# IamJerryXu/Multimodal-Diagnosis-HAM-Spine

Hardware: AMD Instinct MI355X
Metric: training images/sec, ResNet50+BERT-base 224px bs32 (higher is better)
Workload: dtype bf16; 1 GPU; C2: ResNet50 + BERT-base(L=128) + cross-attention FusionModule + MLP head, 224x224, batch 32 per GPU, CE(label_smoothing=0.02), fused AdamW, train-mode BatchNorm and dropout; per_gpu_batch=32, global_batch=32, seq_len=128, params=134897991, parallelism=dp1

## Files before the change

### include/hamspine.h

```cpp
#ifndef HAMSPINE_H
#define HAMSPINE_H

#include <stdint.h>

#ifdef __cplusplus
extern "C" {
#endif

typedef int hs_status;
enum { HS_OK = 0, HS_ERR_ARG = 1, HS_ERR_HIP = 2, HS_ERR_UNSUPPORTED = 3 };
enum { HS_F32 = 0, HS_BF16 = 1 };

const char* hs_last_error(void);
int hs_version(void);
int hs_device_ok(void);


enum {
    HS_A_KC = 0,
    HS_A_RC = 1,
    HS_A_CONV = 2,
    HS_A_DGRAD = 3
};
enum {
// ... 194 lines not shown
                             float* const* exp_avg_sq, const int64_t* n, float lr, float beta1, float beta2, float eps,
                             float weight_decay, int32_t step, int32_t decoupled, float grad_scale, void* stream);
hs_status hs_adam_step_multi_shadow(int32_t count, float* const* params, const float* const* grads, float* const* exp_avg,
                                    float* const* exp_avg_sq, void* const* bf16_shadow, const int64_t* n, float lr, float beta1,
                                    float beta2, float eps, float weight_decay, int32_t step, int32_t decoupled,
                                    float grad_scale, void* stream);
hs_status hs_wgrad_group_begin(void* stream);
hs_status hs_wgrad_group_end(void* stream);
hs_status hs_wgrad_defer_begin(void* stream);
hs_status hs_wgrad_defer_suspend(void* stream);
int32_t hs_wgrad_defer_open(void* stream);
int32_t hs_wgrad_defer_pending(void* stream);
int64_t hs_wgrad_defer_ws_bytes(void* stream);
hs_status hs_wgrad_defer_flush(void* stream, void* ws, int64_t ws_bytes);
hs_status hs_wgrad_defer_abort(void* stream);
void hs_wgrad_defer_counters(int64_t* out);
hs_status hs_weight_shadow_set(const float* w, void* bf16);
void hs_weight_shadow_clear(void);

hs_status hs_sgd_step_multi(int32_t count, float* const* params, const float* const* grads, float* const* momentum_buf,
                            const int64_t* n, float lr, float momentum, float weight_decay, int32_t nesterov, int32_t first,
                            float grad_scale, void* stream);

#define HS_GRADCLIP_MAX 128
hs_status hs_grad_sumsq_multi(int32_t count, const float* const* grads, const int64_t* n, double* partials, void* stream);
int64_t hs_grad_norm_partials(int32_t count, const int64_t* n);
hs_status hs_grad_norm_finish(const double* partials, int64_t n_partials, float max_norm, int32_t skip_nonfinite, float* rec,
                              void* stream);
hs_status hs_grad_scale_multi(int32_t count, float* const* grads, const int64_t* n, const float* rec, void* stream);
hs_status hs_adam_step_multi_clip(int32_t count, float* const* params, const float* const* grads, float* const* exp_avg,
                                  float* const* exp_avg_sq, void* const* bf16_shadow, const int64_t* n, float lr, float beta1,
                                  float beta2, float eps, float weight_decay, int32_t step, int32_t decoupled, float grad_scale,
                                  const float* rec, void* stream);
hs_status hs_sgd_step_multi_clip(int32_t count, float* const* params, const float* const* grads, float* const* momentum_buf,
                                 const int64_t* n, float lr, float momentum, float weight_decay, int32_t nesterov, int32_t first,
                                 float grad_scale, const float* rec, void* stream);

#define HS_MUON_MAX 32
#define HS_MUON_PARTIALS 256
hs_status hs_muon_prepare_multi(int32_t dtype, int32_t count, float* const* momentum, const float* const* grads,
                                void* const* packed, const int32_t* rows, const int32_t* cols, float beta, float* partials,
                                void* stream);
hs_status hs_muon_orthogonalize(int32_t dtype, int32_t count, int32_t rows, int32_t cols, void* X, void* ws, int64_t ws_bytes,
                                void* stream);
int64_t hs_muon_ws_bytes(int32_t dtype, int32_t count, int32_t rows, int32_t cols);
hs_status hs_muon_apply_multi(int32_t dtype, int32_t count, float* const* params, void* const* bf16_shadow,
                              const void* const* packed, const int32_t* rows, const int32_t* cols, const float* scale,
                              float lr, float weight_decay, void* stream);

hs_status hs_select_token_fwd(int32_t dtype, const void* x, float* out, int32_t B, int32_t Nt, int32_t H, int32_t t,
                              void* stream);
hs_status hs_select_token_bwd(int32_t dtype, const float* dy, void* dx, int32_t B, int32_t Nt, int32_t H, int32_t t,
                              void* stream);
hs_status hs_concat2(const float* a, int32_t Ha, const float* b, int32_t Hb, float* out, int64_t rows, void* stream);
hs_status hs_split2(const float* g, float* da, int32_t Ha, float* db, int32_t Hb, int64_t rows, void* stream);
hs_status hs_concat2_t(int32_t dtype, const void* a, int32_t Ha, const void* b, int32_t Hb, void* out, int64_t rows,
                       void* stream);
hs_status hs_split2_t(int32_t dtype, const void* g, void* da, int32_t Ha, void* db, int32_t Hb, int64_t rows, void* stream);
hs_status hs_mul(const float* a, const float* b, float* out, int64_t rows, int32_t cols, int32_t b_mode, void* stream);
hs_status hs_rowdot(const float* a, const float* b, float* out, int32_t rows, int32_t cols, void* stream);
hs_status hs_kl_rows(const float* p, const float* q, float* out, const float* w, float* dp, float* dq, int32_t rows,
                     int32_t cols, float eps, void* stream);
hs_status hs_dot(const float* a, const float* b, float* out, int64_t n, void* stream);
hs_status hs_sigmoid_fwd(const float* x, float* out, int64_t n, void* stream);
hs_status hs_sigmoid_bwd(const float* dy, const float* y, float* dx, int64_t n, void* stream);
hs_status hs_softmax_entropy(const float* logits, const float* g, float* ent, float* dlogits, int32_t rows, int32_t C,
// ... 377 lines not shown
```

### multimodal-diagnosis-ham-spine_amd/hamspine/_lib.py

```python
import collections
import ctypes as C
import os
import re

_HERE = os.path.dirname(os.path.abspath(__file__))
LIB_PATH = os.path.join(_HERE, "libhamspine_hip.so")
HEADER_PATH = os.path.normpath(os.path.join(_HERE, "..", "..", "include", "hamspine.h"))

HS_OK = 0


class HamspineError(RuntimeError):
    pass


_SCALARS = {"int": C.c_int32, "int32_t": C.c_int32, "hs_status": C.c_int32, "int64_t": C.c_int64, "uint64_t": C.c_uint64,
            "float": C.c_float}
_POINTEES = {"void", "char", "double", "uint8_t", "int16_t", "uint16_t", *_SCALARS}

Header = collections.namedtuple("Header", "constants structs prototypes")


def _symbols(text):
    return sorted(set(re.findall(r"\b(hs_[a-z0-9_]+)\s*\(", re.sub(r"/\*.*?\*/", "", text, flags=re.S))))
# ... 120 lines not shown
}
_ALL_STRUCT_NAMES = {**_STRUCT_NAMES, **_LATER_STRUCT_NAMES}
if set(_header.structs) != set(_ALL_STRUCT_NAMES):
    raise HamspineError(f"{HEADER_PATH}: structs without a Python name, or the reverse: {set(_header.structs) ^ set(_ALL_STRUCT_NAMES)}")
_classes = {}
for _c, _fields in _header.structs.items():
    _classes[_c] = type(_ALL_STRUCT_NAMES[_c], (C.Structure,), {"_fields_": [
        (f, _ctype(t, _classes, False) * n if n else _ctype(t, _classes, False)) for f, t, n in _fields]})
globals().update({_ALL_STRUCT_NAMES[_c]: _cls for _c, _cls in _classes.items()})


def abi_structs():
    return list(enumerate(_classes[c] for c in _STRUCT_NAMES))


def later_abi_structs():
    return list(enumerate((_classes[c] for c in _LATER_STRUCT_NAMES), start=len(_STRUCT_NAMES)))


def _const(*names):
    return [_header.constants["HS_" + n] for n in names]


if _const("OK") != [HS_OK]:
    raise HamspineError("HS_OK of the header is not 0")
HS_ERR_ARG, HS_ERR_HIP, HS_ERR_UNSUPPORTED = _const("ERR_ARG", "ERR_HIP", "ERR_UNSUPPORTED")
HS_F32, HS_BF16 = _const("F32", "BF16")
A_KC, A_RC, A_CONV, A_DGRAD = _const("A_KC", "A_RC", "A_CONV", "A_DGRAD")
B_KC, B_RC, B_WDGRAD, B_CONV = _const("B_KC", "B_RC", "B_WDGRAD", "B_CONV")
ACT_NONE, ACT_RELU, ACT_GELU = _const("ACT_NONE", "ACT_RELU", "ACT_GELU")
MUL_NONE, MUL_GELU_GRAD, MUL_RELU_MASK = _const("MUL_NONE", "MUL_GELU_GRAD", "MUL_RELU_MASK")
CAST_MAX, ADAM_MAX, MUON_MAX, MUON_PARTIALS = _const("CAST_MAX", "ADAM_MAX", "MUON_MAX", "MUON_PARTIALS")
GRADCLIP_MAX, = _const("GRADCLIP_MAX")
RESNET_MAX_BLOCKS, RESNET_MAX_TAPS, BERT_MAX_LAYERS = _const("RESNET_MAX_BLOCKS", "RESNET_MAX_TAPS", "BERT_MAX_LAYERS")
JPEG_GEOM, JPEG_CHUNK, JPEG_MAX_COMPONENTS = _const("JPEG_GEOM", "JPEG_CHUNK", "JPEG_MAX_COMPONENTS")
JPEG_STATUS = {v: k[len("HS_JPEG_ERR_"):] for k, v in _header.constants.items() if k.startswith("HS_JPEG_ERR_")}

_lib = None


def lib():
    global _lib
    if _lib is None:
        if not os.path.exists(LIB_PATH):
            raise HamspineError(
                f"{LIB_PATH} not found: build it with `python __graft_entry__.py build` "
                "(hipcc --offload-arch=gfx950). There is no CPU fallback.")
        l = C.CDLL(LIB_PATH)
        missing = [n for n in _header.prototypes if not hasattr(l, n)]
        if missing:
            raise HamspineError(f"{LIB_PATH} lacks declared symbols: {missing}")
        for n, (ret, params) in _header.prototypes.items():
            getattr(l, n).restype = None if ret == "void" else _ctype(ret, _classes, True)
            getattr(l, n).argtypes = [_ctype(t, _classes, True) for t in params]
        _lib = l
    return _lib


def check(status, what=""):
    if status != HS_OK:
        msg = lib().hs_last_error().decode("utf-8", "replace")
        raise HamspineError(f"{what} failed (status {status}): {msg}")
```

### multimodal-diagnosis-ham-spine_amd/hamspine/csrc/elem.hip

```cpp
#include <algorithm>
#include "hs_internal.h"

namespace hs {

static inline int grid_for(long long n, int cap = 4096) {
    long long b = (n + 255) / 256;
    if (b > cap) b = cap;
    if (b < 1) b = 1;
    return (int)b;
}

template <typename T>
__global__ __launch_bounds__(256) void maxpool_fwd_kernel(const T* __restrict__ x, T* __restrict__ y,
                                                          unsigned char* __restrict__ idx, int N, int H, int W, int C,
                                                          int P, int Q, int ks, int st, int pad) {
    constexpr int E = Chunk<T>::N;
    const int cg = C / E;
    const long long total = (long long)N * P * Q * cg;
    for (long long i = (long long)blockIdx.x * 256 + threadIdx.x; i < total; i += (long long)gridDim.x * 256) {
        const int c = (int)(i % cg);
        long long t = i / cg;
        const int q = (int)(t % Q);
        t /= Q;
        const int p = (int)(t % P);
        const int n = (int)(t / P);
        float best[E];
        unsigned char bi[E];
#pragma unroll
        for (int e = 0; e < E; ++e) {
            best[e] = -INFINITY;
            bi[e] = 0;
        }
        for (int r = 0; r < ks; ++r) {
            const int h = p * st - pad + r;
// ... 946 lines not shown
    if (threadIdx.x == 0) loss_out[0] = tn / td;
    if (!dlogits) return;
    for (int r = wv; r < B; r += nwv) {
        const float* z = logits + (long long)r * C;
        float mx = -INFINITY;
        for (int c = lane; c < C; c += 64) mx = fmaxf(mx, z[c]);
        mx = wave_max(mx);
        float se = 0.f;
        for (int c = lane; c < C; c += 64) se += __expf(z[c] - mx);
        const float inv = 1.f / wave_sum(se);
        const int y = (int)labels[r];
        const float wy = weight ? weight[y] : 1.f;
        float wsum = 0.f;
        for (int c = lane; c < C; c += 64) wsum += weight ? weight[c] : 1.f;
        wsum = wave_sum(wsum);
        for (int c = lane; c < C; c += 64) {
            const float p = __expf(z[c] - mx) * inv;
            const float wc = weight ? weight[c] : 1.f;
            float g = (1.f - smoothing) * wy * (p - (c == y ? 1.f : 0.f)) + smoothing / (float)C * (wsum * p - wc);
            dlogits[(long long)r * C + c] = g / td;
        }
    }
}

struct AdamTable {
    float* p[HS_ADAM_MAX];
    const float* g[HS_ADAM_MAX];
    float* m[HS_ADAM_MAX];
    float* v[HS_ADAM_MAX];
    long long n[HS_ADAM_MAX];
    bf16_t* h[HS_ADAM_MAX];
};
__device__ __forceinline__ const float* clip_rec(const float* rec) { return rec; }
template <bool CLIP, typename... Rec>
__global__ __launch_bounds__(256) void adam_multi_kernel(const AdamTable t, float lr, float beta1, float beta2, float eps,
                                                         float wd, float bc1, float bc2_sqrt, int decoupled,
                                                         float grad_scale, Rec... rec) {
    static_assert(sizeof...(Rec) == (CLIP ? 1 : 0), "the record comes with CLIP and only with it");
    float clip = 1.f;
    if constexpr (CLIP) {
        const float* r = clip_rec(rec...);
        if (r[3] != 0.f) return;
        clip = r[1];
    }
    const int e = blockIdx.y;
    float* p = t.p[e];
    const float* g = t.g[e];
    float* m = t.m[e];
    float* v = t.v[e];
    const long long n = t.n[e];
    auto upd = [&](float& pi, float gi, float& mi, float& vi) {
        gi *= grad_scale;
        if constexpr (CLIP) gi *= clip;
        if (decoupled) pi *= 1.f - lr * wd;
        else gi += wd * pi;
        mi = beta1 * mi + (1.f - beta1) * gi;
        vi = beta2 * vi + (1.f - beta2) * gi * gi;
        const float denom = sqrtf(vi) / bc2_sqrt + eps;
        pi = pi - (lr / bc1) * (mi / denom);
    };
    bf16_t* h = t.h[e];
    const bool al = (((uintptr_t)p | (uintptr_t)g | (uintptr_t)m | (uintptr_t)v) & 15) == 0 && (((uintptr_t)h) & 7) == 0;
    const long long n4 = al ? n / 4 : 0;
    for (long long i = (long long)blockIdx.x * 256 + threadIdx.x; i < n4; i += (long long)gridDim.x * 256) {
        f32x4 pv = ((f32x4*)p)[i], mv = ((f32x4*)m)[i], vv = ((f32x4*)v)[i];
        const f32x4 gv = ((const f32x4*)g)[i];
#pragma unroll
        for (int k = 0; k < 4; ++k) {
            float pi = pv[k], mi = mv[k], vi = vv[k];
            upd(pi, gv[k], mi, vi);
            pv[k] = pi; mv[k] = mi; vv[k] = vi;
        }
        ((f32x4*)p)[i] = pv;
        ((f32x4*)m)[i] = mv;
        ((f32x4*)v)[i] = vv;
        if (h) ((bf16x4*)h)[i] = bf16x4{(bf16_t)pv[0], (bf16_t)pv[1], (bf16_t)pv[2], (bf16_t)pv[3]};
    }
    for (long long i = n4 * 4 + (long long)blockIdx.x * 256 + threadIdx.x; i < n; i += (long long)gridDim.x * 256) {
        float pi = p[i], mi = m[i], vi = v[i];
        upd(pi, g[i], mi, vi);
        p[i] = pi; m[i] = mi; v[i] = vi;
        if (h) h[i] = (bf16_t)pi;
    }
}

template <bool CLIP, typename... Rec>
__global__ __launch_bounds__(256) void sgd_multi_kernel(const AdamTable t, float lr, float momentum, float wd, int nesterov,
                                                        int first, float grad_scale, Rec... rec) {
    static_assert(sizeof...(Rec) == (CLIP ? 1 : 0), "the record comes with CLIP and only with it");
    float clip = 1.f;
    if constexpr (CLIP) {
        const float* r = clip_rec(rec...);
        if (r[3] != 0.f) return;
        clip = r[1];
    }
    const int e = blockIdx.y;
    float* p = t.p[e];
    const float* g = t.g[e];
    float* buf = t.m[e];
    const long long n = t.n[e];
    for (long long i = (long long)blockIdx.x * 256 + threadIdx.x; i < n; i += (long long)gridDim.x * 256) {
        float gi = g[i] * grad_scale;
        if constexpr (CLIP) gi *= clip;
        const float pi = p[i];
        if (wd != 0.f) gi += wd * pi;
        if (buf) {
            const float b = first ? gi : momentum * buf[i] + gi;
            buf[i] = b;
            gi = nesterov ? gi + momentum * b : b;
        }
        p[i] = pi - lr * gi;
    }
}

#define DISPATCH_T(dtype, fn, ...) ((dtype) == HS_BF16 ? fn<bf16_t>(__VA_ARGS__) : fn<float>(__VA_ARGS__))
// ... 590 lines not shown
            t.m[i] = exp_avg[base + i];
            t.v[i] = exp_avg_sq[base + i];
            t.n[i] = n[base + i];
            t.h[i] = bf16_shadow ? (bf16_t*)bf16_shadow[base + i] : nullptr;
            mx = std::max<long long>(mx, t.n[i]);
        }
        const int gx = (int)std::min<long long>(std::max<long long>((mx + 4095) / 4096, 1), 256);
        if (rec)
            hipLaunchKernelGGL((adam_multi_kernel<true, const float*>), dim3(gx, cnt), dim3(256), 0, (hipStream_t)stream, t, lr, beta1, beta2, eps,
                               weight_decay, bc1, bc2s, decoupled, grad_scale, rec);
        else
            hipLaunchKernelGGL(adam_multi_kernel<false>, dim3(gx, cnt), dim3(256), 0, (hipStream_t)stream, t, lr, beta1, beta2, eps,
                               weight_decay, bc1, bc2s, decoupled, grad_scale);
        HS_LAUNCH_CHECK();
    }
    return HS_OK;
}
hs_status hs_adam_step_multi_shadow(int32_t count, float* const* params, const float* const* grads, float* const* exp_avg,
                                    float* const* exp_avg_sq, void* const* bf16_shadow, const int64_t* n, float lr, float beta1,
                                    float beta2, float eps, float weight_decay, int32_t step, int32_t decoupled,
                                    float grad_scale, void* stream) {
    return adam_step(count, params, grads, exp_avg, exp_avg_sq, bf16_shadow, n, lr, beta1, beta2, eps, weight_decay, step, decoupled,
                     grad_scale, nullptr, stream);
}
hs_status hs_adam_step_multi_clip(int32_t count, float* const* params, const float* const* grads, float* const* exp_avg,
                                  float* const* exp_avg_sq, void* const* bf16_shadow, const int64_t* n, float lr, float beta1,
                                  float beta2, float eps, float weight_decay, int32_t step, int32_t decoupled, float grad_scale,
                                  const float* rec, void* stream) {
    HS_REQUIRE(rec, "adam_clip: rec is NULL");
    HS_REQUIRE(count <= 0 || (params && grads && exp_avg && exp_avg_sq && n), "adam_clip: NULL table");
    return adam_step(count, params, grads, exp_avg, exp_avg_sq, bf16_shadow, n, lr, beta1, beta2, eps, weight_decay, step, decoupled,
                     grad_scale, rec, stream);
}
}
```

### multimodal-diagnosis-ham-spine_amd/hamspine/csrc/hs_switch.h

```cpp
#pragma once
#include <atomic>
#include <stdlib.h>

namespace hs {
namespace sw {

inline long long off_if_0(const char* e, long long d) { return (e && e[0] == '0') ? 0 : d; }
inline long long on_if_1(const char* e, long long d) { return (e && e[0] == '1') ? 1 : d; }
inline long long int_any(const char* e, long long d) { return e ? atoi(e) : d; }
inline long long int_mask15(const char* e, long long d) { return e ? (atoi(e) & 15) : d; }
inline long long int_1to8(const char* e, long long d) { const long long v = e ? atoi(e) : d; return v >= 1 && v <= 8 ? v : d; }
inline long long int_positive(const char* e, long long d) { const long long v = e ? atoll(e) : 0; return v > 0 ? v : d; }

#define HS_SWITCHES(X) \
   \
  X(p8,                 "HAMSPINE_P8",                  off_if_0,     1,   once,     -, "every GEMM on the generic body, none on the phase-pipelined one") \
  X(p8_wgrad,           "HAMSPINE_P8_WGRAD",            off_if_0,     1,   once,     -, "grouped deep-K weight gradients keep the generic 256x128 tiles") \
  X(conv3,              "HAMSPINE_CONV3",               off_if_0,     1,   once,     -, "3x3 stride-1 convolutions on the generic implicit GEMM, not the halo-patch kernel") \
  X(parity_dgrad,       "HAMSPINE_PARITY_DGRAD",        off_if_0,     1,   once,     -, "stride-2 data gradients keep the natural row order") \
  X(pack_xcd_spread,    "HAMSPINE_PACK_XCD_SPREAD",     off_if_0,     1,   settable, hs_set_pack_xcd_spread, "packed-row launches do not deal their live tiles over all XCDs") \
  X(persistent,         "HAMSPINE_PERSISTENT",          on_if_1,      0,   once,     -, "persistent GEMM launches (measured: no gain)") \
  X(epi_hist,           "HAMSPINE_EPI_HIST",            on_if_1,      0,   once,     -, "measurement: count the epilogue feature sets of the launches, print at exit") \
  X(group_debug,        "HAMSPINE_GROUP_DEBUG",         on_if_1,      0,   once,     -, "measurement: report every upload of a grouped launch's problem table") \
  X(split_units,        "HAMSPINE_SPLIT_UNITS",         int_positive, 512, once,     -, "measurement: the number of workgroups split-K aims at") \
  X(split_max,          "HAMSPINE_SPLIT_MAX",           int_positive, 64,  once,     -, "measurement: the largest split-K factor") \
   \
  X(fused_attention,    "HAMSPINE_FUSED_ATTENTION",     off_if_0,     1,   once,     -, "the unfused attention path") \
   \
  X(overlap,            "HAMSPINE_OVERLAP",             on_if_1,      0,   settable, hs_set_overlap, "a composite's weight gradients run on a side stream beside its data-gradient chain") \
  X(wgrad_nt,           "HAMSPINE_WGRAD_NT",            off_if_0,     1,   settable, hs_set_wgrad_nt, "BertLayer weight gradients from the row-major operands (tn); no packed rows then") \
  X(bert_wgrad_chunks,  "HAMSPINE_BERT_WGRAD_CHUNKS",   off_if_0,     1,   settable, hs_set_bert_wgrad_chunks, "packed text tower: weight gradients walk every padded column") \
  X(grouped_bert_wgrad, "HAMSPINE_GROUPED_BERT_WGRAD",  off_if_0,     1,   once,     -, "every weight-gradient GEMM of a BertLayer on its own") \
  X(wgrad_layers,       "HAMSPINE_WGRAD_LAYERS",        int_1to8,     2,   once,     -, "BERT layers whose weight gradients share one grouped grid (1: flush per layer)") \
  X(dgrad_nt,           "HAMSPINE_DGRAD_NT",            off_if_0,     1,   once,     -, "BERT data gradients read the row-contiguous weights") \
  X(defer_transposes,   "HAMSPINE_DEFER_TRANSPOSES",    off_if_0,     1,   once,     -, "one launch per dY^T where the gradient appears") \
  X(fused_bias_grad,    "HAMSPINE_FUSED_BIAS_GRAD",     off_if_0,     1,   once,     -, "bias gradients by separate column-sum passes") \
  X(fused_ln_bwd,       "HAMSPINE_FUSED_LN_BWD",        off_if_0,     1,   once,     -, "separate LayerNorm-backward / dropout / column-sum passes") \
  X(grouped_wgrad,      "HAMSPINE_GROUPED_WGRAD",       off_if_0,     1,   once,     -, "the image tower backward launches every weight gradient on its own") \
  X(staged_wgrad,       "HAMSPINE_STAGED_WGRAD",        off_if_0,     1,   once,     -, "with gradient milestones, the grouped weight gradients still run only at the end") \
  X(fused_bn_stats,     "HAMSPINE_FUSED_BN_STATS",      off_if_0,     1,   once,     -, "BatchNorm makes its own statistics pass") \
  X(bn_finish,          "HAMSPINE_BN_FINISH",           off_if_0,     1,   once,     -, "BatchNorm finishes its statistics in its own launch") \
  X(fused_bn_bwd,       "HAMSPINE_FUSED_BN_BWD",        off_if_0,     1,   once,     -, "BatchNorm backward makes its own partial-sum pass") \
  X(bnb_finish,         "HAMSPINE_BNB_FINISH",          on_if_1,      0,   once,     -, "the data-gradient GEMM also finishes the BatchNorm-backward sums (measured: no gain)") \
  X(bn_mask_from_x,     "HAMSPINE_BN_MASK_FROM_X",      on_if_1,      0,   once,     -, "inner-stage BatchNorm backward recomputes the ReLU mask from the convolution output (measured neutral)") \
  X(pw_stream,          "HAMSPINE_PW_STREAM",           on_if_1,      0,   once,     -, "1x1 convolutions of a training step through the streaming kernel (measured: a wash)") \
  X(xblock_bn,          "HAMSPINE_XBLOCK_BN",           int_any,      1,   per_call, -, "0: no BatchNorm sums across the block boundary; 2: on every eligible block, whatever its size") \
  X(ds_compact,         "HAMSPINE_DS_COMPACT",          off_if_0,     1,   per_call, -, "bf16 downsample data gradients keep the full-size parity-ordered route") \
  X(img_lean,           "HAMSPINE_IMG_LEAN",            int_mask15,   13,  per_call, -, "bit mask of the bf16 image tower's four lean passes (0: the separate launches)")
#define HS_SWITCHES_MEASURE(X) \
  X(knockout,           "HAMSPINE_KNOCKOUT",            int_any,      0,   once,     -, "bit mask of launch classes left OUT of the step (results are then garbage)")

#define HS_SW_once(id, name, rule, d) \
    inline long long id() { static const long long v = rule(getenv(name), d); return v; }
#define HS_SW_per_call(id, name, rule, d) \
    inline long long id() { return rule(getenv(name), d); }
#define HS_SW_settable(id, name, rule, d)                                                                   \
    inline std::atomic<int>& id##_cell() { static std::atomic<int> v{-1}; return v; }                        \
    inline void set_##id(int on) { id##_cell().store(on ? 1 : 0, std::memory_order_relaxed); }               \
    inline long long id() {                                                                                  \
        int v = id##_cell().load(std::memory_order_relaxed);                                                 \
        if (v < 0) {                                                                                         \
            const int env = (int)rule(getenv(name), d);                                                      \
            if (id##_cell().compare_exchange_strong(v, env, std::memory_order_relaxed)) v = env;             \
        }                                                                                                    \
        return v;                                                                                            \
    }
#define HS_SW_DEFINE(id, name, rule, d, latch, setter, doc) HS_SW_##latch(id, name, rule, d)

HS_SWITCHES(HS_SW_DEFINE)
#ifdef HS_MEASURE
HS_SWITCHES_MEASURE(HS_SW_DEFINE)
#else
constexpr long long knockout() { return 0; }
#endif

}
}
```

### multimodal-diagnosis-ham-spine_amd/hamspine/nn/bert.py

```python
import json
import os
from types import SimpleNamespace

import torch
import torch.nn as nn

import hamspine

from .. import desc as DL
from .. import functional as F
from .layers import Linear, LayerNorm


class BertConfig:
    def __init__(self, vocab_size=30522, hidden_size=768, num_hidden_layers=12, num_attention_heads=12,
                 intermediate_size=3072, hidden_act="gelu", hidden_dropout_prob=0.1, attention_probs_dropout_prob=0.1,
                 max_position_embeddings=512, type_vocab_size=2, layer_norm_eps=1e-12, pad_token_id=0, **unused):
        if hidden_act not in ("gelu",):
            raise ValueError(f"hidden_act={hidden_act!r}: only erf-GELU (BERT's default) is implemented")
        self.vocab_size = vocab_size
        self.hidden_size = hidden_size
        self.num_hidden_layers = num_hidden_layers
        self.num_attention_heads = num_attention_heads
        self.intermediate_size = intermediate_size
        self.hidden_act = hidden_act
        self.hidden_dropout_prob = hidden_dropout_prob
        self.attention_probs_dropout_prob = attention_probs_dropout_prob
        self.max_position_embeddings = max_position_embeddings
        self.type_vocab_size = type_vocab_size
        self.layer_norm_eps = layer_norm_eps
        self.pad_token_id = pad_token_id

    @classmethod
    def from_json_file(cls, path):
        with open(path, "r", encoding="utf-8") as f:
            return cls(**json.load(f))


def _init_linear(m, std=0.02):
    nn.init.normal_(m.weight, mean=0.0, std=std)
    if m.bias is not None:
        nn.init.zeros_(m.bias)


class BertEmbeddings(nn.Module):
    def __init__(self, c):
        super().__init__()
        self.word_embeddings = nn.Embedding(c.vocab_size, c.hidden_size, padding_idx=c.pad_token_id)
        self.position_embeddings = nn.Embedding(c.max_position_embeddings, c.hidden_size)
        self.token_type_embeddings = nn.Embedding(c.type_vocab_size, c.hidden_size)
        self.LayerNorm = LayerNorm(c.hidden_size, eps=c.layer_norm_eps)
        self.dropout = nn.Dropout(c.hidden_dropout_prob)
        for e in (self.word_embeddings, self.position_embeddings, self.token_type_embeddings):
            nn.init.normal_(e.weight, mean=0.0, std=0.02)
        with torch.no_grad():
            self.word_embeddings.weight[c.pad_token_id].zero_()

    def forward(self, input_ids):
        cfg = {"dtype": hamspine.compute_dtype(), "training": self.training, "dropout": float(self.dropout.p),
               "eps": float(self.LayerNorm.eps),
               "pad_id": -1 if self.word_embeddings.padding_idx is None else int(self.word_embeddings.padding_idx)}
        return F.BertEmbedFn.apply(input_ids, cfg, self.word_embeddings.weight, self.position_embeddings.weight,
                                   self.token_type_embeddings.weight, self.LayerNorm.weight, self.LayerNorm.bias)


class BertSelfAttention(nn.Module):
    def __init__(self, c):
        super().__init__()
        self.query = Linear(c.hidden_size, c.hidden_size)
        self.key = Linear(c.hidden_size, c.hidden_size)
        self.value = Linear(c.hidden_size, c.hidden_size)
        self.dropout = nn.Dropout(c.attention_probs_dropout_prob)


class BertSelfOutput(nn.Module):
    def __init__(self, c):
        super().__init__()
        self.dense = Linear(c.hidden_size, c.hidden_size)
        self.LayerNorm = LayerNorm(c.hidden_size, eps=c.layer_norm_eps)
        self.dropout = nn.Dropout(c.hidden_dropout_prob)


class BertAttention(nn.Module):
    def __init__(self, c):
        super().__init__()
        self.self = BertSelfAttention(c)
        self.output = BertSelfOutput(c)


# ... 107 lines not shown
```

### multimodal-diagnosis-ham-spine_amd/hamspine/optim.py

```python
import ctypes as C

import torch

from . import _lib as L
from . import rt


import os as _os
def _knock_adam():
    if not int(_os.environ.get("HAMSPINE_KNOCKOUT", "0")) & 32:
        return False
    return bool(L.lib().hs_measure_build())


_KNOCK_ADAM = None


def _dense(t):
    if t.is_contiguous():
        return True
    expect = 1
    for size, stride in sorted(((s, st) for s, st in zip(t.shape, t.stride()) if s != 1), key=lambda d: d[1]):
        if stride != expect:
            return False
# ... 116 lines not shown
        st["max_grad_norm"], st["nonfinite"] = getattr(self, "max_grad_norm", None), getattr(self, "nonfinite", "propagate")
        return st

    def __setstate__(self, state):
        super().__setstate__(state)
        self._clip_init(self.__dict__.get("max_grad_norm"), self.__dict__.get("nonfinite", "propagate"))

    def _clip_measure(self, grad_scale):
        if grad_scale != 1.0:
            raise L.HamspineError("max_grad_norm together with step(grad_scale != 1) is not supported: the norm is taken of "
                                  ".grad as it stands")
        ps = [p for group in self.param_groups for p in group["params"] if p.grad is not None]
        if not ps:
            return None
        return self._gradnorm.measure(ps, self.max_grad_norm, self._skip_nonfinite)[0]

    def _rec_view(self, i):
        rec = None if getattr(self, "_gradnorm", None) is None else self._gradnorm.rec()
        return None if rec is None else rec[i]

    @property
    def grad_norm(self):
        return self._rec_view(0)

    @property
    def grad_clip_coef(self):
        return self._rec_view(1)

    @property
    def grad_finite(self):
        return self._rec_view(2)


class _FusedAdamBase(_ClipMixin, torch.optim.Optimizer):
    _decoupled = True

    def __init__(self, params, lr=1e-3, betas=(0.9, 0.999), eps=1e-8, weight_decay=0.0, overlap_backward=None,
                 overlap_chunk=8 << 20, max_grad_norm=None, nonfinite="propagate"):
        self._clip_init(max_grad_norm, nonfinite)
        if overlap_backward and self.max_grad_norm is not None:
            raise ValueError("max_grad_norm needs all gradients before the first update: it cannot be combined with "
                             "overlap_backward=True")
        super().__init__(params, dict(lr=lr, betas=betas, eps=eps, weight_decay=weight_decay))
        if overlap_backward is None:
            overlap_backward = _os.environ.get("HAMSPINE_ADAM_OVERLAP", "0") == "1" and self.max_grad_norm is None
        self._overlap = bool(overlap_backward)
        self._chunk = int(_os.environ.get("HAMSPINE_ADAM_CHUNK", "0")) << 20 or int(overlap_chunk)
        self._pending, self._pending_n = [], 0
        self._pending_streams = {}
        self._stream = None
        self._done = set()
        if self._overlap:
            self._group_of = {}
            for g in self.param_groups:
                for p in g["params"]:
                    self._group_of[p] = g
                    p.register_post_accumulate_grad_hook(self._on_grad)

    def _on_grad(self, p):
        if p in self._done:
            raise RuntimeError(
                "FusedAdam(overlap_backward=True): a parameter received a second gradient after its update was enqueued "
                "(a second backward() before step(): gradient accumulation) -- step after backward instead")
        s = torch.cuda.current_stream(p.device)
        self._pending_streams[s.cuda_stream] = s
        if not any(q is p for q in self._pending):
# ... 26 lines not shown
    @torch.no_grad()
    def step(self, closure=None, grad_scale=1.0):
        loss = None
        if closure is not None:
            with torch.enable_grad():
                loss = closure()
        if self._overlap and closure is None and grad_scale == 1.0:
            self._flush()
            done, self._done = self._done, set()
            for group in self.param_groups:
                rest = [p for p in group["params"] if p.grad is not None and p not in done]
                if rest:
                    self._update(group, rest, 1.0)
            if self._stream is not None:
                torch.cuda.current_stream(self._stream.device).wait_stream(self._stream)
            return loss
        rec = self._clip_measure(grad_scale) if getattr(self, "max_grad_norm", None) is not None else None
        for group in self.param_groups:
            ps = [p for p in group["params"] if p.grad is not None]
            if ps:
                self._update(group, ps, grad_scale, rec)
        return loss

    def _update(self, group, ps, grad_scale, rec=None):
        global _KNOCK_ADAM
        if _KNOCK_ADAM is None:
            _KNOCK_ADAM = _knock_adam()
        if not ps or _KNOCK_ADAM:
            return
        lib = L.lib()
        key = (id(group), len(ps), id(ps[0]), id(ps[-1]))
        cache = self.__dict__.setdefault("_tables", {})
        ent = cache.get(key)
        if ent is None or ent["ids"] != [id(p) for p in ps]:
            rt.need_gpu(*ps)
            by_step = {}
            for p in ps:
                st = self.state[p]
                if not st:
                    st["step"] = torch.zeros((), dtype=torch.float32)
                    st["exp_avg"] = torch.zeros_like(p, memory_format=torch.preserve_format)
                    st["exp_avg_sq"] = torch.zeros_like(p, memory_format=torch.preserve_format)
                if p.dtype != torch.float32:
                    raise L.HamspineError("FusedAdam expects f32 parameters and gradients")
                by_step.setdefault(int(st["step"]), []).append(p)
            ent = {"ids": [id(p) for p in ps], "chunks": []}
            for step0, sel in by_step.items():
                n = len(sel)
                arr = lambda ts: (C.c_void_p * n)(*[t.data_ptr() for t in ts])
                shared = torch.tensor(float(step0), dtype=torch.float32)
                for p in sel:
                    self.state[p]["step"] = shared
                ent["chunks"].append({
                    "sel": sel, "n": n, "p": arr(sel), "m": arr([self.state[p]["exp_avg"] for p in sel]),
                    "v": arr([self.state[p]["exp_avg_sq"] for p in sel]), "cnt": (C.c_int64 * n)(*[p.numel() for p in sel]),
                    "ptrs": [p.data_ptr() for p in sel], "strides": [p.stride() for p in sel], "step": shared,
                    "step_host": int(step0), "gptrs": None, "garr": None, "shadow_epoch": -1, "h": None})
            cache[key] = ent
        b1, b2 = group["betas"]
        for ch in ent["chunks"]:
            sel, n = ch["sel"], ch["n"]
            if [p.data_ptr() for p in sel] != ch["ptrs"]:
                cache.pop(key, None)
                return self._update(group, ps, grad_scale, rec)
            gptrs = [p.grad.data_ptr() for p in sel]
            if gptrs != ch["gptrs"]:
                for p, st in zip(sel, ch["strides"]):
                    g = p.grad
                    if g.dtype != torch.float32:
                        raise L.HamspineError("FusedAdam expects f32 parameters and gradients")
                    if g.stride() != st:
                        g2 = torch.empty_like(p, memory_format=torch.preserve_format)
                        g2.copy_(g)
                        p.grad = g2
                gptrs = [p.grad.data_ptr() for p in sel]
                ch["gptrs"], ch["garr"] = gptrs, (C.c_void_p * n)(*gptrs)
            st_all = self.state
            if any(st_all[p]["step"] is not ch["step"] for p in sel):
                cache.pop(key, None)
                return self._update(group, ps, grad_scale, rec)
            ch["step_host"] += 1
            ch["step"].fill_(ch["step_host"])
            if ch["shadow_epoch"] != rt.shadow_epoch():
                hp = [rt.shadow_ptr_of(p) for p in sel]
                ch["h"] = (C.c_void_p * n)(*hp) if any(hp) else None
                ch["shadow_epoch"] = rt.shadow_epoch()
            if rec is not None:
                L.check(lib.hs_adam_step_multi_clip(
                    n, ch["p"], ch["garr"], ch["m"], ch["v"], ch["h"], ch["cnt"], float(group["lr"]), b1, b2, group["eps"],
                    group["weight_decay"], ch["step_host"], 1 if self._decoupled else 0, float(grad_scale), rec.data_ptr(),
                    rt.stream()), "hs_adam_step_multi_clip")
                continue
            L.check(lib.hs_adam_step_multi_shadow(
                n, ch["p"], ch["garr"], ch["m"], ch["v"], ch["h"], ch["cnt"], float(group["lr"]), b1, b2, group["eps"],
                group["weight_decay"], ch["step_host"], 1 if self._decoupled else 0, float(grad_scale), rt.stream()),
                "hs_adam_step_multi_shadow")


class FusedAdamW(_FusedAdamBase):
    _decoupled = True

    def __init__(self, params, lr=1e-3, betas=(0.9, 0.999), eps=1e-8, weight_decay=1e-2, **kw):
        super().__init__(params, lr, betas, eps, weight_decay, **kw)


class FusedAdam(_FusedAdamBase):
    _decoupled = False


class MuonWithAuxAdam(_FusedAdamBase):
    _decoupled = True

    def __init__(self, param_groups):
        groups = []
        for g in param_groups:
            if not isinstance(g, dict) or "use_muon" not in g:
                raise ValueError("MuonWithAuxAdam: every param group needs a `use_muon` entry")
            g = dict(g)
            g["params"] = list(g["params"])
            if g["use_muon"]:
                for k, v in (("lr", 0.02), ("momentum", 0.95), ("weight_decay", 0.0)):
                    g.setdefault(k, v)
                if any(p.ndim < 2 for p in g["params"]):
                    raise ValueError("MuonWithAuxAdam: a use_muon group holds a parameter with ndim < 2")
            else:
                for k, v in (("lr", 3e-4), ("betas", (0.9, 0.95)), ("eps", 1e-10), ("weight_decay", 0.0)):
                    g.setdefault(k, v)
            groups.append(g)
        self._clip_init(None, "propagate")
# ... 162 lines not shown
```

### multimodal-diagnosis-ham-spine_amd/hamspine/rt.py

```python
import ctypes as C
import threading

import torch

from . import _lib as L

_tls = threading.local()
_ws = {}
_seed_lock = threading.Lock()
_seed_state = {"base": None, "ctr": 0}


def stream():
    return C.c_void_p(torch.cuda.current_stream().cuda_stream)


def workspace(nbytes, device):
    key = (device.index if device.index is not None else torch.cuda.current_device(), threading.get_ident(),
           torch.cuda.current_stream().cuda_stream)
    t = _ws.get(key)
    if t is None or t.numel() < nbytes:
        t = torch.empty(max(int(nbytes * 1.25), 1 << 20), dtype=torch.uint8, device=device)
        _ws[key] = t
    return t
# ... 349 lines not shown
        if not ok:
            for p, r in zip(group, recs):
                if r is not None:
                    _forget_shadow(id(p), r.ptr)
            buf = torch.empty(sum(p.numel() for p in group), dtype=torch.bfloat16, device=group[0].device)
            off = 0
            for p in group:
                rec = _Shadow()
                rec.ref, rec.ptr, rec.version, rec.stale = _weakref.ref(p), p.data_ptr(), p._version, True
                rec.view = buf[off:off + p.numel()]
                off += p.numel()
                _shadows[id(p)] = rec
                _shadow_by_ptr[rec.ptr] = id(p)
                L.check(L.lib().hs_weight_shadow_set(rec.ptr, rec.view.data_ptr()), "hs_weight_shadow_set")
                _weakref.finalize(p, _forget_shadow, id(p), rec.ptr)
            _shadow_epoch[0] += 1
            recs = [_shadows[id(p)] for p in group]
        for p, r in zip(group, recs):
            if r.stale or r.version != p._version:
                stale_src.append(p)
                stale_dst.append(r.view)
                r.version, r.stale = p._version, False
    if stale_src:
        n = len(stale_src)
        src = (C.c_void_p * n)(*[t.data_ptr() for t in stale_src])
        dst = (C.c_void_p * n)(*[t.data_ptr() for t in stale_dst])
        cnt = (C.c_int64 * n)(*[t.numel() for t in stale_src])
        L.check(L.lib().hs_cast_f32_to_bf16_multi(n, src, dst, cnt, stream()), "hs_cast_f32_to_bf16_multi")


def clear_shadows():
    for key, rec in list(_shadows.items()):
        _forget_shadow(key, rec.ptr)
```

Measured before the change: 3332 images/s.

## Add row-sparse Adam path for BERT word embeddings skipping untouched rows

Marks the BERT word-embedding table as row-sparse and routes it through a new per-row Adam kernel. Rows whose gradient is zero and whose moments were never populated skip the moment reads and writes and only apply decoupled weight decay. A live-row mask is built once from the moments. This cuts memory traffic for the large vocab table in the optimizer step, at the cost of an extra launch and host-side bookkeeping. The skip is exact only while untouched rows have zero moments.

```diff
diff --git a/include/hamspine.h b/include/hamspine.h
--- a/include/hamspine.h
+++ b/include/hamspine.h
@@ -250,6 +250,16 @@
                                   float* const* exp_avg_sq, void* const* bf16_shadow, const int64_t* n, float lr, float beta1,
                                   float beta2, float eps, float weight_decay, int32_t step, int32_t decoupled, float grad_scale,
                                   const float* rec, void* stream);
+#define HS_ADAM_ROWS_MAX_COLS 1024
+hs_status hs_adam_step_rows(float* param, const float* grad, float* exp_avg, float* exp_avg_sq, void* bf16_shadow, uint8_t* live,
+                            int64_t rows, int64_t cols, float lr, float beta1, float beta2, float eps, float weight_decay,
+                            int32_t step, int32_t decoupled, float grad_scale, void* stream);
+hs_status hs_adam_step_rows_clip(float* param, const float* grad, float* exp_avg, float* exp_avg_sq, void* bf16_shadow, uint8_t* live,
+                                 int64_t rows, int64_t cols, float lr, float beta1, float beta2, float eps, float weight_decay,
+                                 int32_t step, int32_t decoupled, float grad_scale, const float* rec, void* stream);
+hs_status hs_adam_rows_live_from_moments(const float* exp_avg, const float* exp_avg_sq, uint8_t* live, int64_t rows, int64_t cols,
+                                         void* stream);
+int32_t hs_adam_rows_enabled(void);
 hs_status hs_sgd_step_multi_clip(int32_t count, float* const* params, const float* const* grads, float* const* momentum_buf,
                                  const int64_t* n, float lr, float momentum, float weight_decay, int32_t nesterov, int32_t first,
                                  float grad_scale, const float* rec, void* stream);
diff --git a/multimodal-diagnosis-ham-spine_amd/hamspine/_lib.py b/multimodal-diagnosis-ham-spine_amd/hamspine/_lib.py
--- a/multimodal-diagnosis-ham-spine_amd/hamspine/_lib.py
+++ b/multimodal-diagnosis-ham-spine_amd/hamspine/_lib.py
@@ -176,6 +176,7 @@
 MUL_NONE, MUL_GELU_GRAD, MUL_RELU_MASK = _const("MUL_NONE", "MUL_GELU_GRAD", "MUL_RELU_MASK")
 CAST_MAX, ADAM_MAX, MUON_MAX, MUON_PARTIALS = _const("CAST_MAX", "ADAM_MAX", "MUON_MAX", "MUON_PARTIALS")
 GRADCLIP_MAX, = _const("GRADCLIP_MAX")
+ADAM_ROWS_MAX_COLS, = _const("ADAM_ROWS_MAX_COLS")
 RESNET_MAX_BLOCKS, RESNET_MAX_TAPS, BERT_MAX_LAYERS = _const("RESNET_MAX_BLOCKS", "RESNET_MAX_TAPS", "BERT_MAX_LAYERS")
 JPEG_GEOM, JPEG_CHUNK, JPEG_MAX_COMPONENTS = _const("JPEG_GEOM", "JPEG_CHUNK", "JPEG_MAX_COMPONENTS")
 JPEG_STATUS = {v: k[len("HS_JPEG_ERR_"):] for k, v in _header.constants.items() if k.startswith("HS_JPEG_ERR_")}
diff --git a/multimodal-diagnosis-ham-spine_amd/hamspine/csrc/elem.hip b/multimodal-diagnosis-ham-spine_amd/hamspine/csrc/elem.hip
--- a/multimodal-diagnosis-ham-spine_amd/hamspine/csrc/elem.hip
+++ b/multimodal-diagnosis-ham-spine_amd/hamspine/csrc/elem.hip
@@ -1,5 +1,6 @@
 #include <algorithm>
 #include "hs_internal.h"
+#include "hs_switch.h"
 
 namespace hs {
 
@@ -1012,6 +1013,22 @@
     bf16_t* h[HS_ADAM_MAX];
 };
 __device__ __forceinline__ const float* clip_rec(const float* rec) { return rec; }
+template <bool CLIP>
+__device__ __forceinline__ float adam_grad(float gi, float pi, float wd, int decoupled, float grad_scale, float clip) {
+    gi *= grad_scale;
+    if constexpr (CLIP) gi *= clip;
+    if (!decoupled) gi = __builtin_fmaf(wd, pi, gi);
+    return gi;
+}
+__device__ __forceinline__ float adam_decay(float lr, float wd) { return __builtin_fmaf(-lr, wd, 1.f); }
+__device__ __forceinline__ void adam_upd(float& pi, float gi, float& mi, float& vi, float lr, float beta1, float beta2, float eps,
+                                         float wd, float bc1, float bc2_sqrt, int decoupled) {
+    if (decoupled) pi *= adam_decay(lr, wd);
+    mi = __builtin_fmaf(beta1, mi, (1.f - beta1) * gi);
+    vi = __builtin_fmaf(beta2, vi, (1.f - beta2) * gi * gi);
+    const float denom = sqrtf(vi) / bc2_sqrt + eps;
+    pi = pi - (lr / bc1) * (mi / denom);
+}
 template <bool CLIP, typename... Rec>
 __global__ __launch_bounds__(256) void adam_multi_kernel(const AdamTable t, float lr, float beta1, float beta2, float eps,
                                                          float wd, float bc1, float bc2_sqrt, int decoupled,
@@ -1030,14 +1047,8 @@
     float* v = t.v[e];
     const long long n = t.n[e];
     auto upd = [&](float& pi, float gi, float& mi, float& vi) {
-        gi *= grad_scale;
-        if constexpr (CLIP) gi *= clip;
-        if (decoupled) pi *= 1.f - lr * wd;
-        else gi += wd * pi;
-        mi = beta1 * mi + (1.f - beta1) * gi;
-        vi = beta2 * vi + (1.f - beta2) * gi * gi;
-        const float denom = sqrtf(vi) / bc2_sqrt + eps;
-        pi = pi - (lr / bc1) * (mi / denom);
+        gi = adam_grad<CLIP>(gi, pi, wd, decoupled, grad_scale, clip);
+        adam_upd(pi, gi, mi, vi, lr, beta1, beta2, eps, wd, bc1, bc2_sqrt, decoupled);
     };
     bf16_t* h = t.h[e];
     const bool al = (((uintptr_t)p | (uintptr_t)g | (uintptr_t)m | (uintptr_t)v) & 15) == 0 && (((uintptr_t)h) & 7) == 0;
@@ -1061,6 +1072,107 @@
         upd(pi, g[i], mi, vi);
         p[i] = pi; m[i] = mi; v[i] = vi;
         if (h) h[i] = (bf16_t)pi;
+    }
+}
+
+template <int W>
+__device__ __forceinline__ void row_ld(float (&d)[W], const float* s) {
+    if constexpr (W == 4) {
+        const f32x4 t = *(const f32x4*)s;
+        d[0] = t[0]; d[1] = t[1]; d[2] = t[2]; d[3] = t[3];
+    } else {
+        d[0] = *s;
+    }
+}
+template <int W>
+__device__ __forceinline__ void row_st(float* s, const float (&d)[W]) {
+    if constexpr (W == 4) *(f32x4*)s = f32x4{d[0], d[1], d[2], d[3]};
+    else *s = d[0];
+}
+template <int W>
+__device__ __forceinline__ void row_st(bf16_t* s, const float (&d)[W]) {
+    if constexpr (W == 4) *(bf16x4*)s = bf16x4{(bf16_t)d[0], (bf16_t)d[1], (bf16_t)d[2], (bf16_t)d[3]};
+    else *s = (bf16_t)d[0];
+}
+template <bool CLIP, int W, typename... Rec>
+__global__ __launch_bounds__(256) void adam_rows_kernel(float* p, const float* g, float* m, float* v, bf16_t* h, unsigned char* live,
+                                                        int rows, int cols, float lr, float beta1, float beta2, float eps, float wd,
+                                                        float bc1, float bc2_sqrt, int decoupled, float grad_scale, Rec... rec) {
+    static_assert(sizeof...(Rec) == (CLIP ? 1 : 0), "the record comes with CLIP and only with it");
+    constexpr int NC = HS_ADAM_ROWS_MAX_COLS / (64 * W);
+    float clip = 1.f;
+    if constexpr (CLIP) {
+        const float* r = clip_rec(rec...);
+        if (r[3] != 0.f) return;
+        clip = r[1];
+    }
+    const int lane = threadIdx.x & 63;
+    const float decay = adam_decay(lr, wd);
+    for (int row = blockIdx.x * 4 + (threadIdx.x >> 6); row < rows; row += gridDim.x * 4) {
+        const long long base = (long long)row * cols;
+        float gv[NC][W], pv[NC][W];
+#pragma unroll
+        for (int k = 0; k < NC; ++k) {
+            const int c = (k * 64 + lane) * W;
+            if (c < cols) {
+                row_ld<W>(gv[k], g + base + c);
+                row_ld<W>(pv[k], p + base + c);
+            }
+        }
+        bool nz = live[row] != 0;
+#pragma unroll
+        for (int k = 0; k < NC; ++k) {
+            if ((k * 64 + lane) * W < cols) {
+#pragma unroll
+                for (int j = 0; j < W; ++j) {
+                    gv[k][j] = adam_grad<CLIP>(gv[k][j], pv[k][j], wd, decoupled, grad_scale, clip);
+                    nz |= !(gv[k][j] == 0.f);
+                }
+            }
+        }
+        if (__ballot(nz) != 0) {
+#pragma unroll
+            for (int k = 0; k < NC; ++k) {
+                const int c = (k * 64 + lane) * W;
+                if (c < cols) {
+                    float mv[W], vv[W];
+                    row_ld<W>(mv, m + base + c);
+                    row_ld<W>(vv, v + base + c);
+#pragma unroll
+                    for (int j = 0; j < W; ++j) adam_upd(pv[k][j], gv[k][j], mv[j], vv[j], lr, beta1, beta2, eps, wd, bc1, bc2_sqrt, decoupled);
+                    row_st<W>(p + base + c, pv[k]);
+                    row_st<W>(m + base + c, mv);
+                    row_st<W>(v + base + c, vv);
+                    if (h) row_st<W>(h + base + c, pv[k]);
+                }
+            }
+            if (lane == 0) live[row] = 1;
+        } else {
+#pragma unroll
+            for (int k = 0; k < NC; ++k) {
+                const int c = (k * 64 + lane) * W;
+                if (c < cols) {
+                    if (decoupled) {
+#pragma unroll
+                        for (int j = 0; j < W; ++j) pv[k][j] *= decay;
+                    }
+                    row_st<W>(p + base + c, pv[k]);
+                    if (h) row_st<W>(h + base + c, pv[k]);
+                }
+            }
+        }
+    }
+}
+
+__global__ __launch_bounds__(256) void rows_live_from_moments_kernel(const float* m, const float* v, unsigned char* live, int rows,
+                                                                     int cols) {
+    const int lane = threadIdx.x & 63;
+    for (int row = blockIdx.x * 4 + (threadIdx.x >> 6); row < rows; row += gridDim.x * 4) {
+        const long long base = (long long)row * cols;
+        bool nz = false;
+        for (int c = lane; c < cols; c += 64) nz |= m[base + c] != 0.f || v[base + c] != 0.f;
+        const bool any = __ballot(nz) != 0;
+        if (lane == 0) live[row] = any ? 1 : 0;
     }
 }
 
@@ -1717,4 +1829,57 @@
     return adam_step(count, params, grads, exp_avg, exp_avg_sq, bf16_shadow, n, lr, beta1, beta2, eps, weight_decay, step, decoupled,
                      grad_scale, rec, stream);
 }
-}
+
+int32_t hs_adam_rows_enabled(void) { return (int32_t)sw::adam_rows(); }
+static int rows_grid(int64_t rows) { return (int)std::min<int64_t>((rows + 3) / 4, 256 * 5); }
+hs_status hs_adam_rows_live_from_moments(const float* exp_avg, const float* exp_avg_sq, uint8_t* live, int64_t rows, int64_t cols,
+                                         void* stream) {
+    HS_REQUIRE(exp_avg && exp_avg_sq && live, "adam_rows_live: NULL argument");
+    HS_REQUIRE(rows >= 1 && rows <= (1 << 30) && cols >= 1 && cols <= (1 << 30), "adam_rows_live: bad shape");
+    hipLaunchKernelGGL(rows_live_from_moments_kernel, dim3(rows_grid(rows)), dim3(256), 0, (hipStream_t)stream, exp_avg, exp_avg_sq,
+                       live, (int)rows, (int)cols);
+    HS_LAUNCH_CHECK();
+    return HS_OK;
+}
+static int adam_rows(float* p, const float* g, float* m, float* v, void* h, uint8_t* live, int64_t rows, int64_t cols, float lr,
+                     float beta1, float beta2, float eps, float weight_decay, int32_t step, int32_t decoupled, float grad_scale,
+                     const float* rec, void* stream) {
+    HS_REQUIRE(p && g && m && v && live, "adam_rows: NULL argument");
+    HS_REQUIRE(rows >= 1 && rows <= (1 << 30) && cols >= 1 && cols <= HS_ADAM_ROWS_MAX_COLS && step >= 1, "adam_rows: bad argument");
+    HS_REQUIRE((decoupled || weight_decay == 0.f) && eps > 0.f && lr >= 0.f && std::isfinite(lr) && beta1 >= 0.f && beta1 < 1.f &&
+                   beta2 >= 0.f && beta2 < 1.f,
+               "adam_rows: needs decoupled or no weight decay, eps > 0, finite lr >= 0 and betas in [0, 1)");
+    const float bc1 = 1.f - powf(beta1, (float)step);
+    const float bc2s = sqrtf(1.f - powf(beta2, (float)step));
+    const bool vec = cols % 4 == 0 && (((uintptr_t)p | (uintptr_t)g | (uintptr_t)m | (uintptr_t)v) & 15) == 0 && (((uintptr_t)h) & 7) == 0;
+    const dim3 grid(rows_grid(rows)), block(256);
+    hipStream_t s = (hipStream_t)stream;
+#define HS_ROWS_LAUNCH(W)                                                                                                            \
+    do {                                                                                                                             \
+        if (rec)                                                                                                                     \
+            hipLaunchKernelGGL((adam_rows_kernel<true, W, const float*>), grid, block, 0, s, p, g, m, v, (bf16_t*)h, live, (int)rows,  \
+                               (int)cols, lr, beta1, beta2, eps, weight_decay, bc1, bc2s, decoupled, grad_scale, rec);               \
+        else                                                                                                                         \
+            hipLaunchKernelGGL((adam_rows_kernel<false, W>), grid, block, 0, s, p, g, m, v, (bf16_t*)h, live, (int)rows, (int)cols,   \
+                               lr, beta1, beta2, eps, weight_decay, bc1, bc2s, decoupled, grad_scale);                               \
+    } while (0)
+    if (vec) HS_ROWS_LAUNCH(4);
+    else HS_ROWS_LAUNCH(1);
+#undef HS_ROWS_LAUNCH
+    HS_LAUNCH_CHECK();
+    return HS_OK;
+}
+hs_status hs_adam_step_rows(float* param, const float* grad, float* exp_avg, float* exp_avg_sq, void* bf16_shadow, uint8_t* live,
+                            int64_t rows, int64_t cols, float lr, float beta1, float beta2, float eps, float weight_decay,
+                            int32_t step, int32_t decoupled, float grad_scale, void* stream) {
+    return adam_rows(param, grad, exp_avg, exp_avg_sq, bf16_shadow, live, rows, cols, lr, beta1, beta2, eps, weight_decay, step,
+                     decoupled, grad_scale, nullptr, stream);
+}
+hs_status hs_adam_step_rows_clip(float* param, const float* grad, float* exp_avg, float* exp_avg_sq, void* bf16_shadow, uint8_t* live,
+                                 int64_t rows, int64_t cols, float lr, float beta1, float beta2, float eps, float weight_decay,
+                                 int32_t step, int32_t decoupled, float grad_scale, const float* rec, void* stream) {
+    HS_REQUIRE(rec, "adam_rows_clip: rec is NULL");
+    return adam_rows(param, grad, exp_avg, exp_avg_sq, bf16_shadow, live, rows, cols, lr, beta1, beta2, eps, weight_decay, step,
+                     decoupled, grad_scale, rec, stream);
+}
+}
diff --git a/multimodal-diagnosis-ham-spine_amd/hamspine/csrc/hs_switch.h b/multimodal-diagnosis-ham-spine_amd/hamspine/csrc/hs_switch.h
--- a/multimodal-diagnosis-ham-spine_amd/hamspine/csrc/hs_switch.h
+++ b/multimodal-diagnosis-ham-spine_amd/hamspine/csrc/hs_switch.h
@@ -46,7 +46,9 @@
   X(pw_stream,          "HAMSPINE_PW_STREAM",           on_if_1,      0,   once,     -, "1x1 convolutions of a training step through the streaming kernel (measured: a wash)") \
   X(xblock_bn,          "HAMSPINE_XBLOCK_BN",           int_any,      1,   per_call, -, "0: no BatchNorm sums across the block boundary; 2: on every eligible block, whatever its size") \
   X(ds_compact,         "HAMSPINE_DS_COMPACT",          off_if_0,     1,   per_call, -, "bf16 downsample data gradients keep the full-size parity-ordered route") \
-  X(img_lean,           "HAMSPINE_IMG_LEAN",            int_mask15,   13,  per_call, -, "bit mask of the bf16 image tower's four lean passes (0: the separate launches)")
+  X(img_lean,           "HAMSPINE_IMG_LEAN",            int_mask15,   13,  per_call, -, "bit mask of the bf16 image tower's four lean passes (0: the separate launches)") \
+   \
+  X(adam_rows,          "HAMSPINE_ADAM_ROWS",           off_if_0,     1,   per_call, -, "row-sparse tables stay in the dense Adam table: no row-live launch")
 #define HS_SWITCHES_MEASURE(X) \
   X(knockout,           "HAMSPINE_KNOCKOUT",            int_any,      0,   once,     -, "bit mask of launch classes left OUT of the step (results are then garbage)")
 
diff --git a/multimodal-diagnosis-ham-spine_amd/hamspine/nn/bert.py b/multimodal-diagnosis-ham-spine_amd/hamspine/nn/bert.py
--- a/multimodal-diagnosis-ham-spine_amd/hamspine/nn/bert.py
+++ b/multimodal-diagnosis-ham-spine_amd/hamspine/nn/bert.py
@@ -9,6 +9,7 @@
 
 from .. import desc as DL
 from .. import functional as F
+from .. import rt
 from .layers import Linear, LayerNorm
 
 
@@ -55,6 +56,7 @@
             nn.init.normal_(e.weight, mean=0.0, std=0.02)
         with torch.no_grad():
             self.word_embeddings.weight[c.pad_token_id].zero_()
+        rt.mark_row_sparse(self.word_embeddings.weight)
 
     def forward(self, input_ids):
         cfg = {"dtype": hamspine.compute_dtype(), "training": self.training, "dropout": float(self.dropout.p),
diff --git a/multimodal-diagnosis-ham-spine_amd/hamspine/optim.py b/multimodal-diagnosis-ham-spine_amd/hamspine/optim.py
--- a/multimodal-diagnosis-ham-spine_amd/hamspine/optim.py
+++ b/multimodal-diagnosis-ham-spine_amd/hamspine/optim.py
@@ -172,6 +172,17 @@
         return self._rec_view(2)
 
 
+_adam_launches = {"dense": 0, "rows": 0, "rows_live": 0}
+
+
+def adam_launch_counters():
+    return dict(_adam_launches)
+
+
+def _f32(x):
+    return C.c_float(x).value
+
+
 class _FusedAdamBase(_ClipMixin, torch.optim.Optimizer):
     _decoupled = True
 
@@ -264,7 +275,8 @@
         key = (id(group), len(ps), id(ps[0]), id(ps[-1]))
         cache = self.__dict__.setdefault("_tables", {})
         ent = cache.get(key)
-        if ent is None or ent["ids"] != [id(p) for p in ps]:
+        rows_key = (bool(lib.hs_adam_rows_enabled()), rt.row_sparse_epoch())
+        if ent is None or ent["ids"] != [id(p) for p in ps] or ent["rows_key"] != rows_key:
             rt.need_gpu(*ps)
             by_step = {}
             for p in ps:
@@ -276,18 +288,24 @@
                 if p.dtype != torch.float32:
                     raise L.HamspineError("FusedAdam expects f32 parameters and gradients")
                 by_step.setdefault(int(st["step"]), []).append(p)
-            ent = {"ids": [id(p) for p in ps], "chunks": []}
+            ent = {"ids": [id(p) for p in ps], "chunks": [], "rows_key": rows_key}
             for step0, sel in by_step.items():
-                n = len(sel)
-                arr = lambda ts: (C.c_void_p * n)(*[t.data_ptr() for t in ts])
+                rsel = [p for p in sel if rows_key[0] and self._row_table(p)]
+                if rsel:
+                    sel = [p for p in sel if not any(p is q for q in rsel)] + rsel
+                n = len(sel) - len(rsel)
+                arr = lambda ts: (C.c_void_p * len(ts))(*[t.data_ptr() for t in ts])
                 shared = torch.tensor(float(step0), dtype=torch.float32)
                 for p in sel:
                     self.state[p]["step"] = shared
                 ent["chunks"].append({
                     "sel": sel, "n": n, "p": arr(sel), "m": arr([self.state[p]["exp_avg"] for p in sel]),
-                    "v": arr([self.state[p]["exp_avg_sq"] for p in sel]), "cnt": (C.c_int64 * n)(*[p.numel() for p in sel]),
+                    "v": arr([self.state[p]["exp_avg_sq"] for p in sel]),
+                    "cnt": (C.c_int64 * len(sel))(*[p.numel() for p in sel]),
                     "ptrs": [p.data_ptr() for p in sel], "strides": [p.stride() for p in sel], "step": shared,
-                    "step_host": int(step0), "gptrs": None, "garr": None, "shadow_epoch": -1, "h": None})
+                    "step_host": int(step0), "gptrs": None, "garr": None, "shadow_epoch": -1, "h": None, "hp": None,
+                    "rows": [{"i": n + k, "p": p, "live": torch.empty(p.shape[0], dtype=torch.uint8, device=p.device),
+                              "valid": False, "mom": None} for k, p in enumerate(rsel)]})
             cache[key] = ent
         b1, b2 = group["betas"]
         for ch in ent["chunks"]:
@@ -306,7 +324,7 @@
                         g2.copy_(g)
                         p.grad = g2
                 gptrs = [p.grad.data_ptr() for p in sel]
-                ch["gptrs"], ch["garr"] = gptrs, (C.c_void_p * n)(*gptrs)
+                ch["gptrs"], ch["garr"] = gptrs, (C.c_void_p * len(sel))(*gptrs)
             st_all = self.state
             if any(st_all[p]["step"] is not ch["step"] for p in sel):
                 cache.pop(key, None)
@@ -314,19 +332,59 @@
             ch["step_host"] += 1
             ch["step"].fill_(ch["step_host"])
             if ch["shadow_epoch"] != rt.shadow_epoch():
-                hp = [rt.shadow_ptr_of(p) for p in sel]
-                ch["h"] = (C.c_void_p * n)(*hp) if any(hp) else None
+                hp = ch["hp"] = [rt.shadow_ptr_of(p) for p in sel]
+                ch["h"] = (C.c_void_p * len(sel))(*hp) if any(hp) else None
                 ch["shadow_epoch"] = rt.shadow_epoch()
-            if rec is not None:
-                L.check(lib.hs_adam_step_multi_clip(
-                    n, ch["p"], ch["garr"], ch["m"], ch["v"], ch["h"], ch["cnt"], float(group["lr"]), b1, b2, group["eps"],
-                    group["weight_decay"], ch["step_host"], 1 if self._decoupled else 0, float(grad_scale), rec.data_ptr(),
-                    rt.stream()), "hs_adam_step_multi_clip")
-                continue
-            L.check(lib.hs_adam_step_multi_shadow(
-                n, ch["p"], ch["garr"], ch["m"], ch["v"], ch["h"], ch["cnt"], float(group["lr"]), b1, b2, group["eps"],
-                group["weight_decay"], ch["step_host"], 1 if self._decoupled else 0, float(grad_scale), rt.stream()),
-                "hs_adam_step_multi_shadow")
+            lr, eps, wd, dec = float(group["lr"]), group["eps"], group["weight_decay"], 1 if self._decoupled else 0
+            if ch["rows"]:
+                if not ((dec or _f32(wd) == 0.0) and _f32(eps) > 0.0 and 0.0 <= _f32(lr) < float("inf") and
+                        0.0 <= _f32(b1) < 1.0 and 0.0 <= _f32(b2) < 1.0):
+                    n = len(sel)
+                    for r in ch["rows"]:
+                        r["valid"] = False
+            if n:
+                if rec is not None:
+                    L.check(lib.hs_adam_step_multi_clip(
+                        n, ch["p"], ch["garr"], ch["m"], ch["v"], ch["h"], ch["cnt"], lr, b1, b2, eps, wd, ch["step_host"], dec,
+                        float(grad_scale), rec.data_ptr(), rt.stream()), "hs_adam_step_multi_clip")
+                else:
+                    L.check(lib.hs_adam_step_multi_shadow(
+                        n, ch["p"], ch["garr"], ch["m"], ch["v"], ch["h"], ch["cnt"], lr, b1, b2, eps, wd, ch["step_host"], dec,
+                        float(grad_scale), rt.stream()), "hs_adam_step_multi_shadow")
+                _adam_launches["dense"] += (n + L.ADAM_MAX - 1) // L.ADAM_MAX
+            if n < len(sel):
+                for r in ch["rows"]:
+                    self._row_step(r, ch, lr, b1, b2, eps, wd, dec, float(grad_scale), rec)
+
+    def _row_table(self, p):
+        if not rt.is_row_sparse(p) or p.dim() != 2 or p.numel() == 0 or p.shape[1] > L.ADAM_ROWS_MAX_COLS or not p.is_contiguous():
+            return False
+        st = self.state[p]
+        return all(t.dtype == torch.float32 and t.shape == p.shape and t.is_contiguous() and t.device == p.device
+                   for t in (st["exp_avg"], st["exp_avg_sq"]))
+
+    def _row_step(self, r, ch, lr, b1, b2, eps, wd, dec, grad_scale, rec):
+        lib, p, i, s = L.lib(), r["p"], r["i"], rt.stream()
+        st = self.state[p]
+        m, v = st["exp_avg"], st["exp_avg_sq"]
+        mom = (m.data_ptr(), v.data_ptr(), m._version, v._version)
+        if not r["valid"] or mom != r["mom"]:
+            if mom[:2] != (ch["m"][i], ch["v"][i]):
+                if not self._row_table(p):
+                    raise L.HamspineError("FusedAdam: the moments of a row-sparse table were replaced by tensors of another layout")
+                ch["m"][i], ch["v"][i] = mom[0], mom[1]
+            L.check(lib.hs_adam_rows_live_from_moments(mom[0], mom[1], r["live"].data_ptr(), p.shape[0], p.shape[1], s),
+                    "hs_adam_rows_live_from_moments")
+            _adam_launches["rows_live"] += 1
+            r["valid"], r["mom"] = True, mom
+        h = ch["hp"][i] if ch["h"] is not None else None
+        args = (p.data_ptr(), ch["gptrs"][i], mom[0], mom[1], h, r["live"].data_ptr(), p.shape[0], p.shape[1], lr, b1, b2, eps, wd,
+                ch["step_host"], dec, grad_scale)
+        if rec is not None:
+            L.check(lib.hs_adam_step_rows_clip(*args, rec.data_ptr(), s), "hs_adam_step_rows_clip")
+        else:
+            L.check(lib.hs_adam_step_rows(*args, s), "hs_adam_step_rows")
+        _adam_launches["rows"] += 1
 
 
 class FusedAdamW(_FusedAdamBase):
diff --git a/multimodal-diagnosis-ham-spine_amd/hamspine/rt.py b/multimodal-diagnosis-ham-spine_amd/hamspine/rt.py
--- a/multimodal-diagnosis-ham-spine_amd/hamspine/rt.py
+++ b/multimodal-diagnosis-ham-spine_amd/hamspine/rt.py
@@ -405,3 +405,33 @@
 def clear_shadows():
     for key, rec in list(_shadows.items()):
         _forget_shadow(key, rec.ptr)
+
+
+_row_sparse = {}
+_row_sparse_epoch = [0]
+
+
+def _forget_row_sparse(key):
+    ref = _row_sparse.get(key)
+    if ref is not None and ref() is None:
+        del _row_sparse[key]
+
+
+def mark_row_sparse(param):
+    if param.dim() != 2:
+        raise L.HamspineError("mark_row_sparse expects a 2-D parameter")
+    ref = _row_sparse.get(id(param))
+    if ref is not None and ref() is param:
+        return
+    _row_sparse[id(param)] = _weakref.ref(param)
+    _row_sparse_epoch[0] += 1
+    _weakref.finalize(param, _forget_row_sparse, id(param))
+
+
+def is_row_sparse(param):
+    ref = _row_sparse.get(id(param))
+    return ref is not None and ref() is param
+
+
+def row_sparse_epoch():
+    return _row_sparse_epoch[0]
```

Result: no change. 3348 images/s (median of 6 runs) (+0.5%).
